# csukuangfj/kaldi-hmm-gmm

Hardware: AMD Instinct MI355X
Metric: frames/sec (whole node) per EM iter (align+acc-stats), 5k-pdf x 64-Gauss (higher is better)
Workload: dtype f32 via f16x2s

## Files before the change

### include/khg_hip.h

```cpp
#ifndef KHG_HIP_H_
#define KHG_HIP_H_
#include <stdint.h>

#ifdef __cplusplus
extern "C" {
#endif

#define KHG_OK 0
#define KHG_E_ARG (-1)
#define KHG_E_HIP (-2)
#define KHG_E_RUNTIME (-3)
#define KHG_E_UNSUPPORTED (-4)
#define KHG_MAX_DIM 512

typedef struct khg_ctx khg_ctx;
typedef struct khg_model khg_model;
typedef struct khg_tm khg_tm;
typedef struct khg_utts khg_utts;
typedef struct khg_accs khg_accs;

const char *khg_last_error(void);
int khg_version(void);

int khg_ctx_create(int device, void *stream, khg_ctx **out);
// ... 22 lines not shown
#define KHG_OPT_K2_PROF 9
#define KHG_OPT_K3_BUCKET 10
#define KHG_OPT_K3_FORM 11
#define KHG_OPT_K3_PHASE_B 12
#define KHG_OPT_K3_NY 13
#define KHG_OPT_DEBUG 14
#define KHG_OPT_K3_PHASE_A 15
#define KHG_OPT_K2_SPLIT 16
#define KHG_OPT_K2S_HUB 17
#define KHG_OPT_LAT_OPS_LDS 18
#define KHG_OPT_K1_LAUNCH 19
#define KHG_OPT_K1_PGRID 20
#define KHG_OPT_K1_PROF 21
#define KHG_OPT_K2_LADDER 22
#define KHG_OPT_K3_PLANES 23
#define KHG_OPT_COUNT 24
#define KHG_INFO_SCRATCH_BYTES 100
#define KHG_INFO_SCRATCH_BLOCKS 101
int khg_ctx_set_option(khg_ctx *ctx, int option, int value);
int khg_ctx_get_option(const khg_ctx *ctx, int option, int *value);
int khg_option_check(int option, int value);
int khg_option_from_env(const char *name, const char *text, int *option, int *value);

int khg_model_create(khg_ctx *ctx, int32_t num_pdfs, int32_t dim, const int32_t *gauss_off_h,
                     const float *gconsts_h, const float *means_invvars_h,
                     const float *inv_vars_h, khg_model **out);
int khg_model_destroy(khg_model *m);
int khg_model_invalidate(khg_model *m);

int khg_tm_create(khg_ctx *ctx, int32_t num_tids, const int32_t *id2pdf_h, khg_tm **out);
int khg_tm_set_trans_cost(khg_tm *tm, const float *trans_cost_h);
// ... 7 lines not shown
int khg_utts_destroy(khg_utts *u);
typedef struct khg_graph khg_graph;
int khg_graph_create(khg_ctx *ctx, const khg_tm *tm, int32_t num_states, int32_t start, const int64_t *arc_off_h,
                     const int32_t *ilabel_h, const int32_t *olabel_h, const float *weight_h,
                     const int32_t *nextstate_h, const float *final_h, khg_graph **out);
int khg_graph_destroy(khg_graph *g);
int khg_graph_info(const khg_graph *g, int64_t *num_states, int64_t *num_arcs, int32_t *num_pdfs,
                   int32_t *max_in_degree, int64_t *device_bytes);
int khg_utts_create_on_graph(khg_ctx *ctx, const khg_tm *tm, khg_graph *g, int32_t n_utt, int32_t dim,
                             const int64_t *frame_off_h, const float *feats_h, const float *feats_d, khg_utts **out);
int khg_utts_graph_bytes(const khg_utts *u, int64_t *bytes);
int khg_utts_num_pdfs(const khg_utts *u, int64_t *pdf_off_h );
int khg_utts_pdfs(const khg_utts *u, int32_t *pdfs_h );
int khg_utts_k2_plan(khg_ctx *ctx, const khg_utts *u, int32_t out[8]);
int khg_utts_k2_ladder(khg_ctx *ctx, const khg_utts *u, int32_t *out);
int khg_utts_k3_planes(const khg_utts *u, int64_t *bytes, int64_t *packs, int32_t *used);
int khg_utts_pdf_first(const khg_utts *u, int32_t *first_h );

int khg_loglikes(khg_ctx *ctx, const khg_model *m, khg_utts *u);
int khg_loglikes_reachable(khg_ctx *ctx, const khg_model *m, khg_utts *u);
int khg_loglikes_band(khg_ctx *ctx, const khg_model *m, khg_utts *u);
int khg_utts_pdf_last(const khg_utts *u, int32_t *last_h );
int khg_loglikes_layout(const khg_utts *u, int64_t *ll_off_h, int64_t *total);
int khg_loglikes_download(khg_ctx *ctx, const khg_utts *u, float *ll_h);
int khg_loglikes_upload(khg_ctx *ctx, khg_utts *u, const float *ll_h);
int khg_utts_set_pdf_list(khg_utts *u, int32_t n, const int32_t *pdfs_h);
int khg_utts_features_changed(khg_utts *u);

typedef struct {
  float beam;
// ... 460 lines not shown
```

### kaldi_hmm_gmm_amd/_lib.py

```python
import ctypes as C
import os

import numpy as np

_HERE = os.path.dirname(os.path.abspath(__file__))
LIB_PATH = os.environ.get("KHG_LIBRARY") or os.path.join(_HERE, "libkhg_hip.so")


class KhgError(RuntimeError):
    """Mirror of the reference's std::runtime_error -> Python RuntimeError (csrc/log.h:46-53)."""


def _load():
    if not os.path.exists(LIB_PATH):
        raise ImportError(
            f"{LIB_PATH} not found: build it with `python -c 'import __graft_entry__ as g; g.build()'` "
            "(hipcc --offload-arch=gfx950). kaldi_hmm_gmm_amd has no CPU fallback."
        )
    try:
        import torch
    except ImportError:
        pass
    return C.CDLL(LIB_PATH)

# ... 123 lines not shown
        C.c_int,
        [vp, vp, C.c_int32, C.c_int32, c_i64p, c_f32p, vp, c_i64p, c_i32p, c_i64p, c_i32p, c_i32p, c_f32p, c_i32p,
         c_f32p, C.POINTER(vp)],
    ),
    "khg_utts_destroy": (C.c_int, [vp]),
    "khg_graph_create": (C.c_int, [vp, vp, C.c_int32, C.c_int32, c_i64p, c_i32p, c_i32p, c_f32p, c_i32p, c_f32p, C.POINTER(vp)]),
    "khg_graph_destroy": (C.c_int, [vp]),
    "khg_graph_info": (C.c_int, [vp, c_i64p, c_i64p, c_i32p, c_i32p, c_i64p]),
    "khg_utts_create_on_graph": (C.c_int, [vp, vp, vp, C.c_int32, C.c_int32, c_i64p, c_f32p, vp, C.POINTER(vp)]),
    "khg_utts_graph_bytes": (C.c_int, [vp, c_i64p]),
    "khg_utts_num_pdfs": (C.c_int, [vp, c_i64p]),
    "khg_utts_pdfs": (C.c_int, [vp, c_i32p]),
    "khg_utts_k2_plan": (C.c_int, [vp, vp, c_i32p]),
    "khg_utts_k2_ladder": (C.c_int, [vp, vp, c_i32p]),
    "khg_utts_k3_planes": (C.c_int, [vp, c_i64p, c_i64p, c_i32p]),
    "khg_utts_pdf_first": (C.c_int, [vp, c_i32p]),
    "khg_loglikes": (C.c_int, [vp, vp, vp]),
    "khg_loglikes_reachable": (C.c_int, [vp, vp, vp]),
    "khg_loglikes_band": (C.c_int, [vp, vp, vp]),
    "khg_utts_pdf_last": (C.c_int, [vp, c_i32p]),
    "khg_loglikes_layout": (C.c_int, [vp, c_i64p, c_i64p]),
    "khg_loglikes_download": (C.c_int, [vp, vp, c_f32p]),
    "khg_loglikes_upload": (C.c_int, [vp, vp, c_f32p]),
    "khg_utts_set_pdf_list": (C.c_int, [vp, C.c_int32, c_i32p]),
    "khg_utts_features_changed": (C.c_int, [vp]),
    "khg_comm_info": (C.c_int, [vp, c_i32p, c_i32p, c_i32p]),
    "khg_align_config_default": (None, [C.POINTER(AlignConfigC)]),
    "khg_align": (C.c_int, [vp, vp, vp, C.POINTER(AlignConfigC), c_i32p, c_i32p, c_i64p, C.c_int64, c_f32p, c_i32p]),
    "khg_ali_upload": (C.c_int, [vp, vp, c_i32p]),
    "khg_lattice_faster_config_default": (None, [C.POINTER(LatticeFasterConfigC)]),
# ... 203 lines not shown
```

### kaldi_hmm_gmm_amd/csrc/khg_ctx_model.hip

```cpp
#include "khg_internal.hpp"

#include <mutex>
#include "khg_k1_loglikes.hip.inc"

static thread_local std::string g_err;
extern "C" const char* khg_last_error(void) { return g_err.c_str(); }
int khg_set_error(int code, const std::string& msg) { g_err = msg; return code; }
extern "C" int khg_version(void) { return 100; }

static std::mutex g_ctx_mu;
static std::vector<khg_ctx*> g_ctxs;
static constexpr size_t KHG_ARENA_BYTES = size_t(24) << 20;
void* arena_alloc(khg_ctx* ctx, size_t bytes) {
  KhgArena& a = ctx->arena;
  if (!a.dev) {
    if (a.cap == SIZE_MAX) return nullptr;
    void *d = nullptr, *h = nullptr;
    if (hipMalloc(&d, KHG_ARENA_BYTES) != hipSuccess || hipHostMalloc(&h, KHG_ARENA_BYTES, hipHostMallocDefault) != hipSuccess) {
      if (d) (void)hipFree(d);
      (void)hipGetLastError();
      a.cap = SIZE_MAX;
      return nullptr;
    }
    a.dev = static_cast<char*>(d); a.host = static_cast<char*>(h); a.cap = KHG_ARENA_BYTES; a.top = a.base = 256;
// ... 119 lines not shown
  int n = 0; std::string all;
  for (auto& t : c->timings) {
    float v = 0.0f;
    (void)hipEventElapsedTime(&v, t.e0, t.e1);
    if (n < cap && ms) ms[n] = v;
    all += t.name; all += '\n';
    (void)hipEventDestroy(t.e0); (void)hipEventDestroy(t.e1);
    ++n;
  }
  c->timings.clear();
  if (names && names_cap > 0) { size_t k = std::min<size_t>(all.size(), (size_t)names_cap - 1); memcpy(names, all.data(), k); names[k] = 0; }
  *n_out = n;
  return KHG_OK;
}
static const struct { int lo, hi; } k_opt_range[KHG_OPT_COUNT] = {
  {KHG_K1_AUTO, KHG_K1_F16X2S}, {0, 4}, {0, 6}, {0, 1 << 20}, {-1, 1}, {0, 255}, {0, 1}, {0, 4}, {0, 3}, {0, 1}, {0, 2}, {0, 2}, {0, 2}, {0, 64}, {0, 1}, {0, 1}, {0, 1}, {0, 1 << 20}, {0, 1}, {0, 2}, {0, 1 << 16}, {0, 1}, {0, 1}, {0, 2}};
extern "C" int khg_option_check(int opt, int value) {
  if (opt < 0 || opt >= KHG_OPT_COUNT) return khg_set_error(KHG_E_ARG, "khg_option_check: no such option");
  if (value < k_opt_range[opt].lo || value > k_opt_range[opt].hi || (opt == KHG_OPT_K1_FORM && value == 1))
    return khg_set_error(KHG_E_ARG, "khg_ctx_set_option: option " + std::to_string(opt) + " takes values " + std::to_string(k_opt_range[opt].lo) + " .. " + std::to_string(k_opt_range[opt].hi));
  return KHG_OK;
}
extern "C" int khg_ctx_set_option(khg_ctx* c, int opt, int value) {
  if (!c || opt < 0 || opt >= KHG_OPT_COUNT) return khg_set_error(KHG_E_ARG, "khg_ctx_set_option: bad arguments");
  int rc = khg_option_check(opt, value);
  if (rc) return rc;
  c->opt[opt] = value;
  return KHG_OK;
}
extern "C" int khg_ctx_get_option(const khg_ctx* c, int opt, int* value) {
  if (c && value && (opt == KHG_INFO_SCRATCH_BYTES || opt == KHG_INFO_SCRATCH_BLOCKS)) {
// ... 6 lines not shown
}
extern "C" int khg_ctx_set_k1_form(khg_ctx* c, int form) { return khg_ctx_set_option(c, KHG_OPT_K1_FORM, form); }
static const struct { const char* name; int opt; const char* words; } k_env_tab[] = {
  {"KHG_K1", KHG_OPT_K1_FORM, "auto=0,pdf=2,fp32=2,utt=3,f16x2=4,f16x2s=5"},
  {"KHG_K1_ORDER", KHG_OPT_K1_ORDER, "desc=0,none=1,asc=2,tiles=3,xcd=4"},
  {"KHG_K1_NF", KHG_OPT_K1_NF, ""}, {"KHG_K1P_TS", KHG_OPT_K1P_TS, ""}, {"KHG_K1_INTERLEAVE", KHG_OPT_K1_INTERLEAVE, ""},
  {"KHG_K1B_DBG", KHG_OPT_K1_DBG, ""}, {"KHG_K2_INORDER", KHG_OPT_K2_INORDER, ""}, {"KHG_K2_KS", KHG_OPT_K2_KS, ""},
  {"KHG_K2_SERIAL", KHG_OPT_K2_SERIAL, ""}, {"KHG_K2_PROF", KHG_OPT_K2_PROF, ""},
  {"KHG_K3_BUCKET", KHG_OPT_K3_BUCKET, "sort=0,atomic=1,count=2"}, {"KHG_K3_FORM", KHG_OPT_K3_FORM, "auto=0,block=1,valu=2"},
  {"KHG_K3_VALU", KHG_OPT_K3_FORM, "1=2"}, {"KHG_K3_PHASEB", KHG_OPT_K3_PHASE_B, "f64=0,f32=1,f16=2"},
  {"KHG_K3_NY", KHG_OPT_K3_NY, ""}, {"KHG_DEBUG", KHG_OPT_DEBUG, ""}, {"KHG_K3_PHASEA", KHG_OPT_K3_PHASE_A, "auto=0,f16=0,f32=1"},
  {"KHG_K2_SPLIT", KHG_OPT_K2_SPLIT, "on=0,off=1"}, {"KHG_K2S_HUB", KHG_OPT_K2S_HUB, ""},
  {"KHG_LAT_OPS_LDS", KHG_OPT_LAT_OPS_LDS, "on=0,off=1"},
  {"KHG_K1_LAUNCH", KHG_OPT_K1_LAUNCH, "auto=0,chunk=1,persistent=2"}, {"KHG_K1_PGRID", KHG_OPT_K1_PGRID, ""},
  {"KHG_K1_PROF", KHG_OPT_K1_PROF, ""}, {"KHG_K2_LADDER", KHG_OPT_K2_LADDER, "on=0,off=1"},
  {"KHG_K3_PLANES", KHG_OPT_K3_PLANES, "auto=0,off=1,on=2"}};
extern "C" int khg_option_from_env(const char* name, const char* text, int* option, int* value) {
  if (!name || !text || !*text || !option || !value) return khg_set_error(KHG_E_ARG, "khg_option_from_env: bad arguments");
  for (const auto& t : k_env_tab) {
    if (strcmp(t.name, name) != 0) continue;
    const char* e = text;
    int v = atoi(e);
    bool word = false;
    for (const char* w = t.words; *w;) {
      const char* eq = strchr(w, '=');
      const size_t n = (size_t)(eq - w);
      if (strlen(e) == n && strncmp(e, w, n) == 0) { v = atoi(eq + 1); word = true; break; }
      const char* comma = strchr(eq, ',');
      if (!comma) break;
      w = comma + 1;
    }
// ... 339 lines not shown
```

### kaldi_hmm_gmm_amd/csrc/khg_internal.hpp

```cpp
#pragma once
#include <hip/hip_runtime.h>

#include <algorithm>
#include <climits>
#include <cmath>
#include <cstdint>
#include <cstdio>
#include <cstdlib>
#include <cstring>
#include <deque>
#include <limits>
#include <string>
#include <type_traits>
#include <utility>
#include <vector>

#include "../../include/khg_hip.h"
#include "khg_dev_types.hip.inc"

int khg_set_error(int code, const std::string& msg);

#define HIPCHK(expr)                                                                         \
  do {                                                                                       \
    hipError_t e_ = (expr);                                                                  \
// ... 220 lines not shown
  K1sChunk* schunks_d = nullptr; int32_t n_schunks = 0, schunk_nmax = 0;
  K1sUnit* sunits_d = nullptr; std::vector<int32_t> sunits_pto; int sunits_reach = -1;
  uint8_t* bp_d = nullptr; int64_t *bp_off_d = nullptr, *path_off_d = nullptr, *words_off_d = nullptr;
  double* layer_best_d = nullptr; int32_t* layer_cnt_d = nullptr; int32_t* path_d = nullptr;
  unsigned char* k2_gscratch_d = nullptr; size_t k2_gscratch_bytes = 0;
  int32_t* k2_order_d = nullptr;
  int32_t *ali_d = nullptr, *words_d = nullptr, *num_words_d = nullptr, *status_d = nullptr;
  float* like_d = nullptr;
  bool ali_valid = false;
  char* out_blk_d = nullptr; size_t out_blk_bytes = 0;
  hipEvent_t ev_dp = nullptr, ev_ali = nullptr;
  bool ali_pending = false;
  int32_t *ali2_d = nullptr, *unc_d = nullptr, *unc_cnt_h = nullptr, *unc_cnt_dev = nullptr;
  int64_t* sub_off_d = nullptr;
  bool ali_split = false;
  int32_t *pdf_count_d = nullptr, *pdf_cursor_d = nullptr, *frame_ids_d = nullptr;
  uint32_t *sort_keys_d = nullptr, *sort_keys_out_d = nullptr, *sort_vals_d = nullptr; void* sort_tmp_d = nullptr; size_t sort_tmp_bytes = 0;
  int32_t* cs_hist_d = nullptr; size_t cs_hist_n = 0; int64_t* cs_tot_d = nullptr; size_t cs_tot_n = 0;
  double *k3_part_d = nullptr, *k3_llpart_d = nullptr; size_t k3_part_n = 0, k3_llpart_n = 0;
  void* k3_items_d = nullptr; int32_t* k3_item_off_d = nullptr; size_t k3_items_n = 0, k3_item_off_n = 0;
  int64_t* pdf_start_d = nullptr; unsigned long long* tid_count_d = nullptr;
  int32_t k3_P = 0, k3_tids = 0;
  void* k3x_d = nullptr; int64_t k3x_bytes = 0, k3x_packs = 0; std::vector<int32_t> k3x_key; bool k3x_used = false;
  int32_t *pe_row_d = nullptr, *pe_tid_d = nullptr, *pe_ids_d = nullptr; float* pe_w_d = nullptr; size_t pe_cap = 0;
  uint32_t *pe_keys_d = nullptr, *pe_keys_out_d = nullptr, *pe_vals_d = nullptr; void* pe_tmp_d = nullptr; size_t pe_tmp_bytes = 0;
  int64_t* pe_start_d = nullptr; int32_t pe_P = 0;
  uint64_t *rc_keys_d = nullptr, *rc_keys_out_d = nullptr; uint32_t *rc_vals_d = nullptr, *rc_vals_out_d = nullptr;
  int32_t *rc_flag_d = nullptr, *rc_inc_d = nullptr, *rc_row_d = nullptr; float* rc_cell_d = nullptr; size_t rc_cap = 0;
  void* rc_tmp_d = nullptr; size_t rc_tmp_bytes = 0;
  int32_t *rc_cell_start_d = nullptr, *rc_item_off_d = nullptr; int64_t* rc_stats_d = nullptr; int32_t rc_P = -1;
// ... 74 lines not shown
```

### kaldi_hmm_gmm_amd/csrc/khg_k2.hip

```cpp
#include "khg_internal.hpp"

#include "khg_k2_hashlist.hip.inc"
#include "khg_k2_viterbi.hip.inc"

extern "C" void khg_align_config_default(khg_align_config* c) {
  c->beam = 200.0f; c->retry_beam = 0.0f; c->careful = 0; c->acoustic_scale = 1.0f;
  c->max_active = INT32_MAX; c->min_active = 20; c->beam_delta = 0.5f; c->hash_ratio = 2.0f;
  c->like_scale = 0.0f;
}

static int ensure_ali(khg_ctx* ctx, khg_utts* u) {
  if (u->ali_d) return KHG_OK;
  if (u->small && u->has_graphs) {
    const size_t nu = (size_t)u->n_utt, nw = (size_t)u->words_off[u->n_utt];
    const size_t bytes = 4 * (3 * nu + nw + (size_t)u->N) + 64;
    int rc = u_alloc(u, &u->out_blk_d, bytes);
    if (rc) return rc;
    u->out_blk_bytes = bytes;
    int32_t* p = reinterpret_cast<int32_t*>(u->out_blk_d);
    u->status_d = p; u->like_d = reinterpret_cast<float*>(p + nu); u->num_words_d = p + 2 * nu; u->words_d = p + 3 * nu; u->ali_d = p + 3 * nu + nw;
    return KHG_OK;
  }
  return u_alloc(u, &u->ali_d, (size_t)u->N);
}
// ... 82 lines not shown
  if (!u->has_graphs) return khg_set_error(KHG_E_ARG, "khg_utts_k2_plan: the utterance set has no decoding graphs");
  const K2Plan p = k2_plan(ctx, u);
  out[0] = p.KS; out[1] = p.DEG; out[2] = p.FAST ? 1 : 0; out[3] = p.GMEM ? 1 : 0; out[4] = p.SC ? 1 : 0;
  out[5] = p.nthr; out[6] = p.GMEM ? 0 : (int32_t)p.lds_dp; out[7] = p.faithful;
  return KHG_OK;
}

extern "C" int khg_utts_k2_ladder(khg_ctx* ctx, const khg_utts* u, int32_t* out) {
  if (ctx_dead(ctx) || !u || !out) return khg_set_error(KHG_E_ARG, "khg_utts_k2_ladder: bad arguments");
  { int rf = utts_foreign_ctx(ctx, u, "khg_utts_k2_ladder"); if (rf) return rf; }
  if (!u->has_graphs) return khg_set_error(KHG_E_ARG, "khg_utts_k2_ladder: the utterance set has no decoding graphs");
  *out = k2_plan(ctx, u).LAD ? 1 : 0;
  return KHG_OK;
}

extern "C" int khg_align(khg_ctx* ctx, const khg_tm* tm, khg_utts* u, const khg_align_config* cfg,
                         int32_t* ali_h, int32_t* words_h, int64_t* words_off_h, int64_t words_cap,
                         float* like_h, int32_t* status_h) {
  if (ctx_dead(ctx) || !tm || !u || !cfg) return khg_set_error(KHG_E_ARG, "khg_align: bad arguments");
  { int rf = utts_foreign_ctx(ctx, u, "khg_align"); if (rf) return rf; }
  if (!u->has_graphs) return khg_set_error(KHG_E_ARG, "khg_align: the utterance set has no decoding graphs");
  if (!u->ll_valid) return khg_set_error(KHG_E_ARG, "khg_align: call khg_loglikes first");
  if (u->max_states > 65535)
    return khg_set_error(KHG_E_UNSUPPORTED, "khg_align: more than 65535 states in one decoding graph (" + std::to_string(u->max_states) + "); the aligner's limit");
  if (u->max_indeg > 254)
    return khg_set_error(KHG_E_UNSUPPORTED, "khg_align: a state has more than 254 incoming arcs (" + std::to_string(u->max_indeg) + "); the aligner's limit");
  if ((cfg->retry_beam != 0 && cfg->retry_beam <= cfg->beam) || cfg->beam <= 0.0)
    return khg_set_error(KHG_E_RUNTIME, "Beams do not make sense: beam " + std::to_string(cfg->beam) + ", retry-beam " + std::to_string(cfg->retry_beam));
  if (!(cfg->hash_ratio >= 1.0) || !(cfg->max_active > 1) || !(cfg->min_active >= 0 && cfg->min_active < cfg->max_active))
    return khg_set_error(KHG_E_RUNTIME, "FasterDecoderOptions assertion failed");
// ... 16 lines not shown
  }
  rc = arena_flush(ctx);
  if (rc) return rc;
  HIPCHK(hipMemsetAsync(u->ali_d, 0, sizeof(int32_t) * (size_t)u->N, ctx->stream));
  K2Args a;
  a.frame_off = u->frame_off_d; a.gidx = u->gidx_d; a.state_off = u->state_off_d; a.start = u->start_d;
  a.in_off = u->in_off_d; a.in_src = u->in_src_d; a.in_col = u->in_col_d; a.in_tid = u->in_tid_d;
  a.in_olabel = u->in_olabel_d; a.in_w = u->in_w_d; a.out_off = u->out_off_d; a.out_inidx = u->out_inidx_d;
  a.final_w = u->final_d; a.trans_cost = tm->has_trans_cost ? tm->trans_cost_d : nullptr;
  a.ll = u->ll_d; a.ll_off = u->ll_off_d;
  a.bp = u->bp_d; a.bp_off = u->bp_off_d; a.layer_best = u->layer_best_d; a.layer_cnt = u->layer_cnt_d;
  a.path = u->path_d; a.path_off = u->path_off_d;
  a.ali = u->ali_d; a.ali_fb = u->ali_d; a.unc = nullptr; a.unc_cnt = nullptr; a.words = u->words_d; a.words_off = u->words_off_d; a.num_words = u->num_words_d;
  a.like = u->like_d; a.status = u->status_d; a.err_flag = ctx->err_flag_d;
  a.prof = nullptr;
  if (!u->k2_order_d && u->n_utt > 1) {
    std::vector<int32_t> ord((size_t)u->n_utt);
    for (int i = 0; i < u->n_utt; ++i) ord[(size_t)i] = i;
    std::stable_sort(ord.begin(), ord.end(), [&](int32_t x, int32_t y) {
      return u->frame_off[x + 1] - u->frame_off[x] > u->frame_off[y + 1] - u->frame_off[y];
    });
    int rc2 = u_upload(ctx, u, &u->k2_order_d, ord);
    if (!rc2) rc2 = sync_pageable(ctx);
    if (rc2) return rc2;
  }
  a.order = ctx->opt[KHG_OPT_K2_INORDER] ? nullptr : u->k2_order_d;
  const bool split = !(ali_h || like_h || status_h || words_h) && u->n_utt > 64 && !u->small && ctx->opt[KHG_OPT_K2_SPLIT] == 0;
  if (split) {
    if (!u->ali2_d) {
      rc = u_alloc(u, &u->ali2_d, (size_t)u->N);
// ... 91 lines not shown
      if (plan.lds_f > 48 * 1024) HIPCHK(hipFuncSetAttribute((const void*)k2_viterbi_faithful<false>, hipFuncAttributeMaxDynamicSharedMemorySize, (int)plan.lds_f));
      KHG_LAUNCH(ctx, k2_viterbi_faithful<false>, dim3(u->n_utt), dim3(64), plan.lds_f, side, a);
    }
  }
  HIPCHK(hipGetLastError());
  if (!sync_call) { HIPCHK(hipEventRecord(u->ev_ali, side)); u->ali_pending = true; }
  u->ali_split = split;
  u->ali_valid = true;
  if (k2prof) {
    std::vector<long long> pr(16 * (size_t)u->n_utt);
    HIPCHK(hipStreamSynchronize(ctx->stream));
    HIPCHK(hipStreamSynchronize(side));
    HIPCHK(hipMemcpy(pr.data(), a.prof, pr.size() * 8, hipMemcpyDeviceToHost));
    (void)hipFree(a.prof);
    double ph[4] = {0, 0, 0, 0}, sT = 0, sS = 0, sf = 0; int n = 0;
    for (int i = 0; i < u->n_utt; ++i) if (pr[i * 8 + 4]) { for (int k = 0; k < 4; ++k) ph[k] += (double)(pr[i * 8 + k + 1] - pr[i * 8 + k]); sT += pr[i * 8 + 5]; sS += pr[i * 8 + 6]; sf += pr[i * 8 + 7]; ++n; }
    if (n) fprintf(stderr, "[KHG_K2_PROF] %d utts, avg T %.1f S %.1f fast %.2f threads %d lds %zu | ticks: setup %.0f forward %.0f traceback %.0f replay %.0f\n",
                   n, sT / n, sS / n, sf / n, nthr, lds_dp, ph[0] / n, ph[1] / n, ph[2] / n, ph[3] / n);
    const long long* pc = pr.data() + 8 * (size_t)u->n_utt;
    double cs[3] = {0, 0, 0}, cf = 0, cp[3] = {0, 0, 0}; int nc = 0;
    for (int i = 0; i < u->n_utt; ++i) if (pc[i * 8 + 3]) { for (int k = 0; k < 3; ++k) { cs[k] += (double)(pc[i * 8 + k + 1] - pc[i * 8 + k]); cp[k] += (double)pc[i * 8 + 5 + k]; } cf += (double)pc[i * 8 + 4]; ++nc; }
    if (nc) fprintf(stderr, "[KHG_K2_PROF] chain decoder: %d utts, avg frames decoded %.1f | ticks: setup %.0f frames %.0f (%.1f per frame: GetCutoff %.1f, pass 1 %.1f, pass 2 %.1f, rest = row flush + score staging) finish %.0f\n",
                    nc, cf / nc, cs[0] / nc, cs[1] / nc, cs[1] / std::max(1.0, cf), cp[0] / std::max(1.0, cf), cp[1] / std::max(1.0, cf), cp[2] / std::max(1.0, cf), cs[2] / nc);
  }
  if (!ali_h && !like_h && !status_h && !words_h) return KHG_OK;
  rc = wait_ali(ctx, u);
  if (rc) return rc;
  if (u->out_blk_d && ctx->arena.owns(u->out_blk_d)) {
    char* hm = ctx->arena.mirror(u->out_blk_d);
    HIPCHK(hipMemcpyAsync(hm, u->out_blk_d, u->out_blk_bytes, hipMemcpyDeviceToHost, ctx->stream));
    rc = check_err_flag(ctx, "khg_align");
    if (rc) return rc;
    const size_t nu = (size_t)u->n_utt, nwt = (size_t)u->words_off[u->n_utt];
// ... 72 lines not shown
```

### kaldi_hmm_gmm_amd/csrc/khg_k2_viterbi.hip.inc

```

struct K2Args {
  const int64_t* frame_off;
  const int32_t* gidx;
  const int64_t* state_off;
  const int32_t* start;
  const int64_t* in_off;
  const int32_t* in_src;
  const int32_t* in_col;
  const int32_t* in_tid;
  const int32_t* in_olabel;
  const float* in_w;
  const int64_t* out_off;
  const int32_t* out_inidx;
  const float* final_w;
  const float* trans_cost;
  const float* ll;
  const int64_t* ll_off;
  uint8_t* bp;
  const int64_t* bp_off;
  double* layer_best;
  int32_t* layer_cnt;
  int32_t* path;
  const int64_t* path_off;
  int32_t* ali;
// ... 1 lines not shown
  int32_t* unc;
  int32_t* unc_cnt;
  int32_t* words;
  const int64_t* words_off;
  int32_t* num_words;
  float* like;
  int32_t* status;
  int32_t* err_flag;
  long long* prof;
  float beam, retry_beam, acoustic_scale, like_scale, beam_delta, hash_ratio;
  int32_t max_active, min_active;
  int32_t max_states, max_inarcs;
  unsigned char* gscratch;
  int64_t gscratch_stride;
  const int32_t* order;
};

#ifndef K2_WAVES_PER_EU
#define K2_WAVES_PER_EU 5
#endif
#define K2_BP_NONE 255
#define K2_ST_NEED_FALLBACK 16

__device__ __forceinline__ unsigned long long k2_d2key(double d) {
  unsigned long long b = (unsigned long long)__double_as_longlong(d);
  return (b & 0x8000000000000000ull) ? ~b : (b | 0x8000000000000000ull);
}
__device__ __forceinline__ double k2_key2d(unsigned long long k) {
  unsigned long long b = (k & 0x8000000000000000ull) ? (k & 0x7fffffffffffffffull) : ~k;
  return __longlong_as_double((long long)b);
}

__device__ int k2_finish(const K2Args& a, int u, int best_state, const int32_t* s_in_off,
                         const int32_t* s_src, const int32_t* s_col, const float* s_w,
// ... 92 lines not shown
               "v_min_f32_dpp %0, %0, %0 row_bcast:15 row_mask:0xa bank_mask:0xf\n\ts_nop 1\n\t"
               "v_min_f32_dpp %0, %0, %0 row_bcast:31 row_mask:0xc bank_mask:0xf\n\ts_nop 1"
               : "+v"(v));
  return v;
}
__device__ __forceinline__ double k2_wave_min(double v) {
#pragma unroll
  for (int o = 32; o > 0; o >>= 1) { double t = __shfl_xor(v, o); v = t < v ? t : v; }
  return v;
}
template <int CTRL, int ROWMASK>
__device__ __forceinline__ double k2_dpp_d(double old, double v) {
  const int lo = __builtin_amdgcn_update_dpp(__double2loint(old), __double2loint(v), CTRL, ROWMASK, 0xf, false);
  const int hi = __builtin_amdgcn_update_dpp(__double2hiint(old), __double2hiint(v), CTRL, ROWMASK, 0xf, false);
  return __hiloint2double(hi, lo);
}
__device__ __forceinline__ int k2_wave_sum(int v) {
#pragma unroll
  for (int o = 32; o > 0; o >>= 1) v += __shfl_xor(v, o);
  return v;
}
__device__ __forceinline__ float k2_round_down(double d) {
  float f = (float)d;
  if ((double)f > d) f = __int_as_float(__float_as_int(f) + (f > 0.0f ? -1 : (f < 0.0f ? 1 : (int)0x80000001)));
  return f;
}

template <int DEG, int NB>
__device__ __forceinline__ void k2_decode_nibble(int nib, int& ord, int& tie) {
  if constexpr (DEG == 2) { ord = (nib & 1) ? 0 : ((nib & 2) ? 1 : (1 << NB) - 1); tie = (nib & 3) == 3 ? 1 : 0; }
// ... 471 lines not shown
      const unsigned* W = reinterpret_cast<const unsigned*>(bp);
      const uint32_t* arcw = reinterpret_cast<const uint32_t*>(s_arc);
      auto trace = [&](auto nslot_c) {
        constexpr int NSLOT = decltype(nslot_c)::value;
        int ioff[NSLOT];
        unsigned w[NSLOT], wn[NSLOT];
        int g = T >> 3;
#pragma unroll
        for (int q = 0; q < NSLOT; ++q) {
          const int sq = lane + 64 * q;
          ioff[q] = sq < S ? s_in_off[sq] : 0;
          w[q] = W[(int64_t)g * GW + min(sq, GW - 1)];
          wn[q] = 0u;
        }
        int sst = __builtin_amdgcn_readfirstlane(st);
        for (; g >= 0 && !bad; --g) {
          if (g > 0) {
#pragma unroll
            for (int q = 0; q < NSLOT; ++q) wn[q] = W[(int64_t)(g - 1) * GW + min(lane + 64 * q, GW - 1)];
          }
          int aiv[8][NSLOT], srcv[8][NSLOT];
#pragma unroll
          for (int k = 0; k < 8; ++k)
#pragma unroll
            for (int q = 0; q < NSLOT; ++q) {
              const int nib = (int)((w[q] >> (4 * k)) & 15u);
              int ord, tieb;
              k2_decode_nibble<DEG, NB>(nib, ord, tieb);
              const int none = ord == BNONE;
              const int ai = ioff[q] + (none ? 0 : ord);
// ... 86 lines not shown
      }
      hi = layer < 0 ? -1 : lo;
    }
    hi = __shfl(hi, 0); st = __shfl(st, 0); n = __shfl(n, 0); bad = __shfl(bad, 0); ptie = __shfl(ptie, 0);
    k2_lds_sync();
  }
  if (a.prof && tid == 0) a.prof[u * 8 + 3] = clock64();
  double cost = 0.0;
  float v1 = 0.0f, v2 = 0.0f;
  int t = 0, nw = 0;
  bool ok = !bad;
  const double beam = (double)a.beam;
  const int64_t wcap = a.words_off[u + 1] - a.words_off[u];
  int32_t* words = a.words + a.words_off[u];
  k2_global_sync();
  if (!bad) {
    ok = (0.0 < lbest[0] + beam) || lcnt[0] <= a.min_active;
    for (int base = n - 1; base >= 0; base -= 64) {
      const int idx = base - lane;
      int ai = 0, col = -1, tidl = 0, ol = 0; float w = 0.0f, ac = 0.0f;
      if (idx >= 0) {
        ai = path[idx];
        K2Arc ar = s_arc[ai];
        col = ar.col; w = ar.w;
        tidl = a.in_tid[in0 + ai];
        ol = a.in_olabel[in0 + ai];
      }
      const unsigned long long em = __ballot(idx >= 0 && col >= 0);
      const int before = __popcll(em & ((1ull << lane) - 1ull));
      const int tf = t + before;
      if (idx >= 0 && col >= 0) {
        ac = -1 * (a.acoustic_scale * llu[(int64_t)col * tpad + tf]);
        a.ali[f0 + tf] = tidl;
// ... 21 lines not shown
      const float tot_cost = (float)(ca - cb);
      const float ac_cost = tot_cost - w;
      if (__ballot(mine && !(ca < lb) && !small) != 0ull) ok = false;
      t += __popcll(em);
      {
        const unsigned long long wm = __ballot(mine && ol != 0);
        if (mine && ol != 0) { const int pos = nw + __popcll(wm & ((1ull << lane) - 1ull)); if (pos < wcap) words[pos] = ol; }
        nw += __popcll(wm);
      }
      for (int k = 0; k < cnt; ++k) {
        v1 = __int_as_float(__builtin_amdgcn_readlane(__float_as_int(w), k)) + v1;
        v2 = __int_as_float(__builtin_amdgcn_readlane(__float_as_int(ac_cost), k)) + v2;
      }
    }
  }
  if (a.prof && tid == 0) { a.prof[u * 8 + 4] = clock64(); a.prof[u * 8 + 5] = T; a.prof[u * 8 + 6] = S; a.prof[u * 8 + 7] = FAST; }
  int stt = 0;
  if (lane == 0) {
    if (bad || nw > wcap) {
      stt = K2_ST_NEED_FALLBACK;
    } else {
      v1 = a.final_w[s0 + best_state] + v1;
      v2 = 0.0f + v2;
      a.num_words[u] = nw;
      a.like[u] = -(v1 + v2) / a.like_scale;
      stt = (ok && !tie && !ptie && a.max_active == INT32_MAX) ? (KHG_ALIGN_DONE | KHG_ALIGN_EXACT_DP) : K2_ST_NEED_FALLBACK;
    }
    a.status[u] = stt;
  }
  if (a.unc) {
    stt = __builtin_amdgcn_readfirstlane(stt);
// ... 1140 lines not shown
```

### kaldi_hmm_gmm_amd/csrc/khg_pybind.cpp

```cpp
#include <chrono>

#include <pybind11/numpy.h>
#include <pybind11/pybind11.h>
#include <pybind11/stl.h>

#include <cstdint>
#include <cstring>
#include <limits>
#include <string>
#include <vector>

#include "../../include/khg_hip.h"
#include "khg_py_ebw.hpp"
#include "khg_py_lattices.hpp"

namespace py = pybind11;

namespace {

py::object g_khg_error;

void Check(int rc) {
  if (rc == KHG_OK) return;
  const char* msg = khg_last_error();
// ... 27 lines not shown
    void* st = stream.is_none() ? nullptr : reinterpret_cast<void*>(stream.cast<uintptr_t>());
    Check(khg_ctx_create(dev, st, &h));
  }
  ~KContext() { close(); }
  void close() { if (h) { khg_ctx_destroy(h); h = nullptr; } }
  void sync() { Check(NoGil([&] { return khg_ctx_sync(h); })); }
  void set_timing(bool on) { Check(khg_ctx_set_timing(h, on ? 1 : 0)); }
  void set_k1_form(const std::string& f) {
    int v = f == "auto" ? KHG_K1_AUTO : (f == "pdf" || f == "fp32") ? KHG_K1_FP32_PDF : f == "utt" ? KHG_K1_FP32_UTT : f == "f16x2" ? KHG_K1_F16X2 : f == "f16x2s" ? KHG_K1_F16X2S : -1;
    if (v < 0) throw py::key_error(f);
    Check(khg_ctx_set_k1_form(h, v));
  }
  static int opt_id(const py::object& o) {
    if (py::isinstance<py::int_>(o)) return o.cast<int>();
    static const char* names[KHG_OPT_COUNT] = {"k1_form", "k1_order", "k1_nf", "k1p_ts", "k1_interleave", "k1_dbg", "k2_inorder", "k2_ks", "k2_serial",
                                               "k2_prof", "k3_bucket", "k3_form", "k3_phase_b", "k3_ny", "debug", "k3_phase_a", "k2_split", "k2s_hub", "lat_ops_lds", "k1_launch", "k1_pgrid", "k1_prof", "k2_ladder", "k3_planes"};
    const std::string n = o.cast<std::string>();
    for (int i = 0; i < KHG_OPT_COUNT; ++i) if (n == names[i]) return i;
    if (n == "scratch_bytes") return KHG_INFO_SCRATCH_BYTES;
    if (n == "scratch_blocks") return KHG_INFO_SCRATCH_BLOCKS;
    throw py::key_error(n);
  }
  int get_option(py::object name) { int v = 0; Check(khg_ctx_get_option(h, opt_id(name), &v)); return v; }
  int set_option(py::object name, int value) {
    const int id = opt_id(name);
    int old = 0;
    Check(khg_ctx_get_option(h, id, &old));
    Check(khg_ctx_set_option(h, id, value));
    return old;
  }
  py::list timings() {
// ... 557 lines not shown
    d["nthr"] = o[5]; d["lds_bytes"] = o[6]; d["faithful_form"] = o[7];
    return d;
  }
  py::dict k3_planes() {
    int64_t bytes = 0, packs = 0; int32_t used = 0;
    Check(khg_utts_k3_planes(h, &bytes, &packs, &used));
    py::dict d;
    d["bytes"] = bytes; d["packs"] = packs; d["used"] = used != 0;
    return d;
  }
  bool k2_ladder(py::object ctx_o) {
    int32_t o = 0;
    Check(khg_utts_k2_ladder(ctx_o.cast<KContext*>()->h, h, &o));
    return o != 0;
  }
  py::object pdf_first_frames() {
    Arr<int64_t> off({(py::ssize_t)n_utt + 1});
    Check(khg_utts_num_pdfs(h, off.mutable_data()));
    const py::ssize_t n = off.at(n_utt);
    Arr<int32_t> first({n > 0 ? n : 1});
    Check(khg_utts_pdf_first(h, first.mutable_data()));
    return py::array(first)[py::slice(0, n, 1)];
  }
  py::object pdf_last_frames() {
    Arr<int64_t> off({(py::ssize_t)n_utt + 1});
    Check(khg_utts_num_pdfs(h, off.mutable_data()));
    const py::ssize_t n = off.at(n_utt);
    Arr<int32_t> last({n > 0 ? n : 1});
    Check(khg_utts_pdf_last(h, last.mutable_data()));
    return py::array(last)[py::slice(0, n, 1)];
// ... 395 lines not shown
      .def("allreduce_range", &KAccs::allreduce_range, py::arg("model"), py::arg("first_pdf"), py::arg("n_pdf"), py::arg("comm") = py::none())
      .def("split", &KAccs::split).def("relayout", &KAccs::relayout).def("download_range", &KAccs::download_range)
      .def("download_occ", [](KAccs& a) { return a.download_range(0, a.sumG); })
      .def("download_trans", &KAccs::download_trans).def("download", &KAccs::download).def("upload", &KAccs::upload)
      .def("add", &KAccs::add, py::arg("scale"), py::arg("src")).def("scale", &KAccs::scale, py::arg("f"))
      .def("smooth_with_accum", &KAccs::smooth_with_accum, py::arg("tau"), py::arg("src"), py::arg("model"), py::arg("count") = true)
      .def("close", &KAccs::close);

  py::class_<KUtts>(m, "UtteranceSet")
      .def(py::init<py::object, py::object, Arr<int64_t>, py::object, py::object, py::object, py::object>(), py::arg("ctx"), py::arg("tm"), py::arg("frame_off"),
           py::arg("feats"), py::arg("dim") = py::none(), py::arg("graphs") = py::none(), py::arg("graph") = py::none())
      .def_property_readonly("graph_bytes", [](KUtts& x) { int64_t b = 0; Check(khg_utts_graph_bytes(x.h, &b)); return b; })
      .def_property_readonly("h", [](KUtts& x) { return reinterpret_cast<uintptr_t>(x.h); })
      .def_readonly("ctx", &KUtts::ctx_obj).def_readonly("frame_off", &KUtts::frame_off).def_readonly("n_utt", &KUtts::n_utt)
      .def_readonly("dim", &KUtts::dim)
      .def("set_pdf_list", &KUtts::set_pdf_list).def("features_changed", &KUtts::features_changed).def("pdf_lists", &KUtts::pdf_lists).def("k2_plan", &KUtts::k2_plan, py::arg("ctx")).def("k2_ladder", &KUtts::k2_ladder, py::arg("ctx")).def("k3_planes", &KUtts::k3_planes).def("pdf_first_frames", &KUtts::pdf_first_frames)
      .def("pdf_last_frames", &KUtts::pdf_last_frames)
      .def("loglikes", &KUtts::loglikes, py::arg("model"), py::arg("reachable_only") = false, py::arg("band") = false)
      .def("loglikes_layout", &KUtts::loglikes_layout).def("download_loglikes", &KUtts::download_loglikes)
      .def("upload_loglikes", &KUtts::upload_loglikes)
      .def("align", &KUtts::align, py::arg("tm"), py::arg("beam") = 200.0f, py::arg("retry_beam") = 0.0f, py::arg("acoustic_scale") = 1.0f,
           py::arg("careful") = false, py::arg("max_active") = (int64_t)std::numeric_limits<int32_t>::max(), py::arg("min_active") = 20,
           py::arg("beam_delta") = 0.5f, py::arg("hash_ratio") = 2.0f, py::arg("download") = true)
      .def("decode_lattice_faster", &KUtts::decode_lattice_faster, py::arg("tm"), py::arg("beam") = 16.0f,
           py::arg("max_active") = std::numeric_limits<int32_t>::max(), py::arg("min_active") = 200, py::arg("lattice_beam") = 10.0f,
           py::arg("prune_interval") = 25, py::arg("beam_delta") = 0.5f, py::arg("hash_ratio") = 2.0f, py::arg("prune_scale") = 0.1f,
           py::arg("acoustic_scale") = 1.0f, py::arg("allow_partial") = true, py::arg("scratch_per_frame") = 0)
      .def("raw_lattice_faster", &KUtts::raw_lattice_faster, py::arg("tm"), py::arg("beam") = 16.0f,
           py::arg("max_active") = std::numeric_limits<int32_t>::max(), py::arg("min_active") = 200, py::arg("lattice_beam") = 10.0f,
           py::arg("prune_interval") = 25, py::arg("beam_delta") = 0.5f, py::arg("hash_ratio") = 2.0f, py::arg("prune_scale") = 0.1f,
           py::arg("acoustic_scale") = 1.0f, py::arg("allow_partial") = true, py::arg("scratch_per_frame") = 0)
// ... 281 lines not shown
```

Before: 449.2 million.

## Parallelize Viterbi traceback and replay cost accumulation with wave scans

Adds a branch-free traceback path for low in-degree graphs that precomputes source-state words per lane and walks 8 frames per word with readlane, avoiding per-frame LDS lookups. It also replaces the lane-serial cost replay with a wave-wide double prefix scan. The scan runs only when an exponent/magnitude bound shows the reassociated sum matches the serial float order, and otherwise falls back to the serial loop. Both paths are on by default and can be disabled with a new KHG_K2_TAIL option. Profiling now reports how many replay batches took the scanned path versus the serial one.

```diff
diff --git a/include/khg_hip.h b/include/khg_hip.h
--- a/include/khg_hip.h
+++ b/include/khg_hip.h
@@ -60,7 +60,8 @@
 #define KHG_OPT_K1_PROF 21
 #define KHG_OPT_K2_LADDER 22
 #define KHG_OPT_K3_PLANES 23
-#define KHG_OPT_COUNT 24
+#define KHG_OPT_K2_TAIL 24
+#define KHG_OPT_COUNT 25
 #define KHG_INFO_SCRATCH_BYTES 100
 #define KHG_INFO_SCRATCH_BLOCKS 101
 int khg_ctx_set_option(khg_ctx *ctx, int option, int value);
@@ -98,6 +99,7 @@
 int khg_utts_pdfs(const khg_utts *u, int32_t *pdfs_h );
 int khg_utts_k2_plan(khg_ctx *ctx, const khg_utts *u, int32_t out[8]);
 int khg_utts_k2_ladder(khg_ctx *ctx, const khg_utts *u, int32_t *out);
+int khg_utts_k2_tail(const khg_utts *u, int32_t *out, int64_t cap);
 int khg_utts_k3_planes(const khg_utts *u, int64_t *bytes, int64_t *packs, int32_t *used);
 int khg_utts_pdf_first(const khg_utts *u, int32_t *first_h );
 
diff --git a/kaldi_hmm_gmm_amd/_lib.py b/kaldi_hmm_gmm_amd/_lib.py
--- a/kaldi_hmm_gmm_amd/_lib.py
+++ b/kaldi_hmm_gmm_amd/_lib.py
@@ -161,6 +161,7 @@
     "khg_utts_k2_plan": (C.c_int, [vp, vp, c_i32p]),
     "khg_utts_k2_ladder": (C.c_int, [vp, vp, c_i32p]),
     "khg_utts_k3_planes": (C.c_int, [vp, c_i64p, c_i64p, c_i32p]),
+    "khg_utts_k2_tail": (C.c_int, [vp, c_i32p, C.c_int64]),
     "khg_utts_pdf_first": (C.c_int, [vp, c_i32p]),
     "khg_loglikes": (C.c_int, [vp, vp, vp]),
     "khg_loglikes_reachable": (C.c_int, [vp, vp, vp]),
diff --git a/kaldi_hmm_gmm_amd/csrc/khg_ctx_model.hip b/kaldi_hmm_gmm_amd/csrc/khg_ctx_model.hip
--- a/kaldi_hmm_gmm_amd/csrc/khg_ctx_model.hip
+++ b/kaldi_hmm_gmm_amd/csrc/khg_ctx_model.hip
@@ -157,7 +157,7 @@
   return KHG_OK;
 }
 static const struct { int lo, hi; } k_opt_range[KHG_OPT_COUNT] = {
-  {KHG_K1_AUTO, KHG_K1_F16X2S}, {0, 4}, {0, 6}, {0, 1 << 20}, {-1, 1}, {0, 255}, {0, 1}, {0, 4}, {0, 3}, {0, 1}, {0, 2}, {0, 2}, {0, 2}, {0, 64}, {0, 1}, {0, 1}, {0, 1}, {0, 1 << 20}, {0, 1}, {0, 2}, {0, 1 << 16}, {0, 1}, {0, 1}, {0, 2}};
+  {KHG_K1_AUTO, KHG_K1_F16X2S}, {0, 4}, {0, 6}, {0, 1 << 20}, {-1, 1}, {0, 255}, {0, 1}, {0, 4}, {0, 3}, {0, 1}, {0, 2}, {0, 2}, {0, 2}, {0, 64}, {0, 1}, {0, 1}, {0, 1}, {0, 1 << 20}, {0, 1}, {0, 2}, {0, 1 << 16}, {0, 1}, {0, 1}, {0, 2}, {0, 1}};
 extern "C" int khg_option_check(int opt, int value) {
   if (opt < 0 || opt >= KHG_OPT_COUNT) return khg_set_error(KHG_E_ARG, "khg_option_check: no such option");
   if (value < k_opt_range[opt].lo || value > k_opt_range[opt].hi || (opt == KHG_OPT_K1_FORM && value == 1))
@@ -194,7 +194,7 @@
   {"KHG_LAT_OPS_LDS", KHG_OPT_LAT_OPS_LDS, "on=0,off=1"},
   {"KHG_K1_LAUNCH", KHG_OPT_K1_LAUNCH, "auto=0,chunk=1,persistent=2"}, {"KHG_K1_PGRID", KHG_OPT_K1_PGRID, ""},
   {"KHG_K1_PROF", KHG_OPT_K1_PROF, ""}, {"KHG_K2_LADDER", KHG_OPT_K2_LADDER, "on=0,off=1"},
-  {"KHG_K3_PLANES", KHG_OPT_K3_PLANES, "auto=0,off=1,on=2"}};
+  {"KHG_K3_PLANES", KHG_OPT_K3_PLANES, "auto=0,off=1,on=2"}, {"KHG_K2_TAIL", KHG_OPT_K2_TAIL, "on=0,off=1"}};
 extern "C" int khg_option_from_env(const char* name, const char* text, int* option, int* value) {
   if (!name || !text || !*text || !option || !value) return khg_set_error(KHG_E_ARG, "khg_option_from_env: bad arguments");
   for (const auto& t : k_env_tab) {
diff --git a/kaldi_hmm_gmm_amd/csrc/khg_internal.hpp b/kaldi_hmm_gmm_amd/csrc/khg_internal.hpp
--- a/kaldi_hmm_gmm_amd/csrc/khg_internal.hpp
+++ b/kaldi_hmm_gmm_amd/csrc/khg_internal.hpp
@@ -258,6 +258,7 @@
   int32_t *ali2_d = nullptr, *unc_d = nullptr, *unc_cnt_h = nullptr, *unc_cnt_dev = nullptr;
   int64_t* sub_off_d = nullptr;
   bool ali_split = false;
+  std::vector<int32_t> k2_tail;
   int32_t *pdf_count_d = nullptr, *pdf_cursor_d = nullptr, *frame_ids_d = nullptr;
   uint32_t *sort_keys_d = nullptr, *sort_keys_out_d = nullptr, *sort_vals_d = nullptr; void* sort_tmp_d = nullptr; size_t sort_tmp_bytes = 0;
   int32_t* cs_hist_d = nullptr; size_t cs_hist_n = 0; int64_t* cs_tot_d = nullptr; size_t cs_tot_n = 0;
diff --git a/kaldi_hmm_gmm_amd/csrc/khg_k2.hip b/kaldi_hmm_gmm_amd/csrc/khg_k2.hip
--- a/kaldi_hmm_gmm_amd/csrc/khg_k2.hip
+++ b/kaldi_hmm_gmm_amd/csrc/khg_k2.hip
@@ -120,6 +120,14 @@
   return KHG_OK;
 }
 
+extern "C" int khg_utts_k2_tail(const khg_utts* u, int32_t* out, int64_t cap) {
+  if (!u || !out) return khg_set_error(KHG_E_ARG, "khg_utts_k2_tail: bad arguments");
+  if (u->k2_tail.empty()) return khg_set_error(KHG_E_ARG, "khg_utts_k2_tail: no khg_align under KHG_OPT_K2_PROF on this set yet");
+  if (cap < (int64_t)u->k2_tail.size()) return khg_set_error(KHG_E_ARG, "khg_utts_k2_tail: cap too small");
+  std::copy(u->k2_tail.begin(), u->k2_tail.end(), out);
+  return KHG_OK;
+}
+
 extern "C" int khg_align(khg_ctx* ctx, const khg_tm* tm, khg_utts* u, const khg_align_config* cfg,
                          int32_t* ali_h, int32_t* words_h, int64_t* words_off_h, int64_t words_cap,
                          float* like_h, int32_t* status_h) {
@@ -166,6 +174,7 @@
   a.ali = u->ali_d; a.ali_fb = u->ali_d; a.unc = nullptr; a.unc_cnt = nullptr; a.words = u->words_d; a.words_off = u->words_off_d; a.num_words = u->num_words_d;
   a.like = u->like_d; a.status = u->status_d; a.err_flag = ctx->err_flag_d;
   a.prof = nullptr;
+  a.tail_off = ctx->opt[KHG_OPT_K2_TAIL];
   if (!u->k2_order_d && u->n_utt > 1) {
     std::vector<int32_t> ord((size_t)u->n_utt);
     for (int i = 0; i < u->n_utt; ++i) ord[(size_t)i] = i;
@@ -287,9 +296,15 @@
     HIPCHK(hipMemcpy(pr.data(), a.prof, pr.size() * 8, hipMemcpyDeviceToHost));
     (void)hipFree(a.prof);
     double ph[4] = {0, 0, 0, 0}, sT = 0, sS = 0, sf = 0; int n = 0;
-    for (int i = 0; i < u->n_utt; ++i) if (pr[i * 8 + 4]) { for (int k = 0; k < 4; ++k) ph[k] += (double)(pr[i * 8 + k + 1] - pr[i * 8 + k]); sT += pr[i * 8 + 5]; sS += pr[i * 8 + 6]; sf += pr[i * 8 + 7]; ++n; }
-    if (n) fprintf(stderr, "[KHG_K2_PROF] %d utts, avg T %.1f S %.1f fast %.2f threads %d lds %zu | ticks: setup %.0f forward %.0f traceback %.0f replay %.0f\n",
-                   n, sT / n, sS / n, sf / n, nthr, lds_dp, ph[0] / n, ph[1] / n, ph[2] / n, ph[3] / n);
+    for (int i = 0; i < u->n_utt; ++i) if (pr[i * 8 + 4]) { for (int k = 0; k < 4; ++k) ph[k] += (double)(pr[i * 8 + k + 1] - pr[i * 8 + k]); sT += pr[i * 8 + 5]; sS += pr[i * 8 + 6]; sf += (double)(pr[i * 8 + 7] & 0xff); ++n; }
+    u->k2_tail.assign(2 * (size_t)u->n_utt, 0);
+    long long bs = 0, bl = 0;
+    for (int i = 0; i < u->n_utt; ++i) {
+      u->k2_tail[2 * (size_t)i] = (int32_t)((pr[i * 8 + 7] >> 8) & 0xffffff); u->k2_tail[2 * (size_t)i + 1] = (int32_t)(pr[i * 8 + 7] >> 32);
+      bs += u->k2_tail[2 * (size_t)i]; bl += u->k2_tail[2 * (size_t)i + 1];
+    }
+    if (n) fprintf(stderr, "[KHG_K2_PROF] %d utts, avg T %.1f S %.1f fast %.2f threads %d lds %zu | ticks: setup %.0f forward %.0f traceback %.0f replay %.0f | replay batches: %lld scanned, %lld serial\n",
+                   n, sT / n, sS / n, sf / n, nthr, lds_dp, ph[0] / n, ph[1] / n, ph[2] / n, ph[3] / n, bs, bl);
     const long long* pc = pr.data() + 8 * (size_t)u->n_utt;
     double cs[3] = {0, 0, 0}, cf = 0, cp[3] = {0, 0, 0}; int nc = 0;
     for (int i = 0; i < u->n_utt; ++i) if (pc[i * 8 + 3]) { for (int k = 0; k < 3; ++k) { cs[k] += (double)(pc[i * 8 + k + 1] - pc[i * 8 + k]); cp[k] += (double)pc[i * 8 + 5 + k]; } cf += (double)pc[i * 8 + 4]; ++nc; }
diff --git a/kaldi_hmm_gmm_amd/csrc/khg_k2_viterbi.hip.inc b/kaldi_hmm_gmm_amd/csrc/khg_k2_viterbi.hip.inc
--- a/kaldi_hmm_gmm_amd/csrc/khg_k2_viterbi.hip.inc
+++ b/kaldi_hmm_gmm_amd/csrc/khg_k2_viterbi.hip.inc
@@ -39,10 +39,17 @@
   unsigned char* gscratch;
   int64_t gscratch_stride;
   const int32_t* order;
+  int32_t tail_off;
 };
 
 #ifndef K2_WAVES_PER_EU
 #define K2_WAVES_PER_EU 5
+#endif
+#ifndef K2_TAIL_TRACE
+#define K2_TAIL_TRACE 1
+#endif
+#ifndef K2_TAIL_REPLAY
+#define K2_TAIL_REPLAY 1
 #endif
 #define K2_BP_NONE 255
 #define K2_ST_NEED_FALLBACK 16
@@ -165,6 +172,28 @@
   const int lo = __builtin_amdgcn_update_dpp(__double2loint(old), __double2loint(v), CTRL, ROWMASK, 0xf, false);
   const int hi = __builtin_amdgcn_update_dpp(__double2hiint(old), __double2hiint(v), CTRL, ROWMASK, 0xf, false);
   return __hiloint2double(hi, lo);
+}
+__device__ __forceinline__ double k2_wave_scand(double v) {
+  v += k2_dpp_d<0x111, 0xf>(0.0, v);
+  v += k2_dpp_d<0x112, 0xf>(0.0, v);
+  v += k2_dpp_d<0x114, 0xf>(0.0, v);
+  v += k2_dpp_d<0x118, 0xf>(0.0, v);
+  v += k2_dpp_d<0x142, 0xa>(0.0, v);
+  v += k2_dpp_d<0x143, 0xc>(0.0, v);
+  return v;
+}
+__device__ __forceinline__ double k2_readlane_d(double v, int l) {
+  return __hiloint2double(__builtin_amdgcn_readlane(__double2hiint(v), l), __builtin_amdgcn_readlane(__double2loint(v), l));
+}
+__device__ __forceinline__ double k2_wave_sumd(double v) { return k2_readlane_d(k2_wave_scand(v), 63); }
+__device__ __forceinline__ unsigned k2_wave_minu(unsigned v) {
+  v = min(v, (unsigned)__builtin_amdgcn_update_dpp(-1, (int)v, 0x111, 0xf, 0xf, false));
+  v = min(v, (unsigned)__builtin_amdgcn_update_dpp(-1, (int)v, 0x112, 0xf, 0xf, false));
+  v = min(v, (unsigned)__builtin_amdgcn_update_dpp(-1, (int)v, 0x114, 0xf, 0xf, false));
+  v = min(v, (unsigned)__builtin_amdgcn_update_dpp(-1, (int)v, 0x118, 0xf, 0xf, false));
+  v = min(v, (unsigned)__builtin_amdgcn_update_dpp(-1, (int)v, 0x142, 0xa, 0xf, false));
+  v = min(v, (unsigned)__builtin_amdgcn_update_dpp(-1, (int)v, 0x143, 0xc, 0xf, false));
+  return (unsigned)__builtin_amdgcn_readlane((int)v, 63);
 }
 __device__ __forceinline__ int k2_wave_sum(int v) {
 #pragma unroll
@@ -666,6 +695,66 @@
           wn[q] = 0u;
         }
         int sst = __builtin_amdgcn_readfirstlane(st);
+        if constexpr (K2_TAIL_TRACE && DEG <= 3 && KS == 1) {
+          if (!a.tail_off) {
+            constexpr int NBITS = NB + 1;
+            int srcr[NSLOT][DEG], srcx[NSLOT][DEG];
+#pragma unroll
+            for (int q = 0; q < NSLOT; ++q) {
+              const int sq = lane + 64 * q;
+              const int ib = sq < S ? s_in_off[sq] : 0, ie = sq < S ? s_in_off[sq + 1] : 0;
+#pragma unroll
+              for (int j = 0; j < DEG; ++j) srcr[q][j] = ib + j < ie ? (int)((arcw[2 * (ib + j)] & 0xffffu) << NBITS) : 0;
+#pragma unroll
+              for (int j = 0; j + 1 < DEG; ++j) srcx[q][j] = srcr[q][j] ^ srcr[q][DEG - 1];
+            }
+            for (; g >= 0 && !bad; --g) {
+              if (g > 0) {
+#pragma unroll
+                for (int q = 0; q < NSLOT; ++q) wn[q] = W[(int64_t)(g - 1) * GW + min(lane + 64 * q, GW - 1)];
+              }
+              int pk[8][NSLOT];
+#pragma unroll
+              for (int k = 0; k < 8; ++k)
+#pragma unroll
+                for (int q = 0; q < NSLOT; ++q) {
+                  const int nib = (int)((w[q] >> (4 * k)) & (unsigned)((1 << NBITS) - 1));
+                  int sel = srcr[q][0];
+                  if constexpr (DEG == 2) sel = srcr[q][1] ^ (srcx[q][0] & -(nib & 1));
+                  if constexpr (DEG == 3) { const int o = nib & BNONE; sel = srcr[q][2] ^ (srcx[q][0] & -(int)(o == 0)) ^ (srcx[q][1] & -(int)(o == 1)); }
+                  pk[k][q] = sel | nib;
+                }
+              int pv = 0, cnt = 0;
+#pragma unroll
+              for (int k = 7; k >= 0; --k) {
+                const int L = 8 * g + k;
+                if (L <= T && L >= 1 && !bad) {
+                  const int q = sst >> 6, l = sst & 63;
+                  int pw = __builtin_amdgcn_readlane(pk[k][0], l);
+#pragma unroll
+                  for (int qq = 1; qq < NSLOT; ++qq)
+                    if (q == qq) pw = __builtin_amdgcn_readlane(pk[k][qq], l);
+                  int ord, tieb;
+                  k2_decode_nibble<DEG, NB>(pw & ((1 << NBITS) - 1), ord, tieb);
+                  if (ord == BNONE) {
+                    bad = 1;
+                  } else {
+                    ptie |= tieb;
+                    pv = lane == cnt ? ((sst << NBITS) | ord) : pv;
+                    ++cnt;
+                    sst = pw >> NBITS;
+                  }
+                }
+              }
+              if (lane < cnt) path[n + lane] = s_in_off[pv >> NBITS] + (pv & BNONE);
+              n += cnt;
+#pragma unroll
+              for (int q = 0; q < NSLOT; ++q) w[q] = wn[q];
+            }
+            st = sst;
+            return;
+          }
+        }
         for (; g >= 0 && !bad; --g) {
           if (g > 0) {
 #pragma unroll
@@ -782,9 +871,88 @@
   const int64_t wcap = a.words_off[u + 1] - a.words_off[u];
   int32_t* words = a.words + a.words_off[u];
   k2_global_sync();
-  if (!bad) {
+  int nscan = 0, nserial = 0;
+  bool replayed = false;
+  if constexpr (FAST && K2_TAIL_REPLAY) {
+    if (!bad && !a.tail_off) {
+      replayed = true;
+      ok = (0.0 < lbest[0] + beam) || lcnt[0] <= a.min_active;
+      unsigned emin1 = 0xffffffffu;
+      double sumabs = 0.0;
+      bool serial = false;
+      f32x2 vv = {0.0f, 0.0f};
+      for (int base = n - 1; base >= 0; base -= 64) {
+        const int idx = base - lane;
+        const bool mine = idx >= 0;
+        int ai = 0, col = 0, tidl = 0, ol = 0; float w = 0.0f, ac = 0.0f;
+        if (mine) {
+          ai = path[idx];
+          K2Arc ar = s_arc[ai];
+          col = ar.col; w = ar.w;
+          tidl = a.in_tid[in0 + ai];
+          ol = a.in_olabel[in0 + ai];
+        }
+        const int tf = t + lane;
+        if (mine) {
+          ac = -1 * (a.acoustic_scale * llu[(int64_t)col * tpad + tf]);
+          a.ali[f0 + tf] = tidl;
+        }
+        const int cnt = base >= 63 ? 64 : base + 1;
+        const int tl = tf + (mine ? 1 : 0);
+        double lb = 0.0; int small = 0;
+        if (mine) {
+          lb = lbest[tl] + beam;
+          small = lcnt[tl] <= a.min_active && (tl == 0 || lcnt[tl - 1] <= a.min_active);
+        }
+        const double cost_in = cost;
+        double ca = 0.0;
+        if (!serial) {
+          const unsigned aw = __float_as_uint(w) & 0x7fffffffu, aa = __float_as_uint(ac) & 0x7fffffffu;
+          const unsigned m1 = k2_wave_minu(min(aw - 1u, aa - 1u));
+          emin1 = min(emin1, m1);
+          sumabs += k2_wave_sumd((double)__uint_as_float(aw) + (double)__uint_as_float(aa));
+          const unsigned eb = (emin1 + 1u) >> 23;
+          const double bound = __hiloint2double((int)((eb + 925u) << 20), 0);
+          serial = !((emin1 == 0xffffffffu || eb >= 27u) && sumabs <= bound);
+        }
+        if (!serial) {
+          ++nscan;
+          double d = (double)w + (double)ac;
+          d = lane == 0 ? cost_in + d : d;
+          ca = k2_wave_scand(d);
+          cost = k2_readlane_d(ca, cnt - 1);
+        } else {
+          ++nserial;
+          for (int k = 0; k < cnt; ++k) {
+            const float wk = __int_as_float(__builtin_amdgcn_readlane(__float_as_int(w), k));
+            const float ack = __int_as_float(__builtin_amdgcn_readlane(__float_as_int(ac), k));
+            const double ncost = (cost + wk) + ack;
+            ca = lane == k ? ncost : ca;
+            cost = ncost;
+          }
+        }
+        const double cb = k2_dpp_d<0x138, 0xf>(cost_in, ca);
+        const float tot_cost = (float)(ca - cb);
+        const float ac_cost = tot_cost - w;
+        if (__ballot(mine && !(ca < lb) && !small) != 0ull) ok = false;
+        t += cnt;
+        {
+          const unsigned long long wm = __ballot(mine && ol != 0);
+          if (mine && ol != 0) { const int pos = nw + __popcll(wm & ((1ull << lane) - 1ull)); if (pos < wcap) words[pos] = ol; }
+          nw += __popcll(wm);
+        }
+        for (int k = 0; k < cnt; ++k) {
+          const f32x2 r = {__int_as_float(__builtin_amdgcn_readlane(__float_as_int(w), k)), __int_as_float(__builtin_amdgcn_readlane(__float_as_int(ac_cost), k))};
+          vv = r + vv;
+        }
+      }
+      v1 = vv[0]; v2 = vv[1];
+    }
+  }
+  if (!bad && !replayed) {
     ok = (0.0 < lbest[0] + beam) || lcnt[0] <= a.min_active;
     for (int base = n - 1; base >= 0; base -= 64) {
+      ++nserial;
       const int idx = base - lane;
       int ai = 0, col = -1, tidl = 0, ol = 0; float w = 0.0f, ac = 0.0f;
       if (idx >= 0) {
@@ -836,7 +1004,7 @@
       }
     }
   }
-  if (a.prof && tid == 0) { a.prof[u * 8 + 4] = clock64(); a.prof[u * 8 + 5] = T; a.prof[u * 8 + 6] = S; a.prof[u * 8 + 7] = FAST; }
+  if (a.prof && tid == 0) { a.prof[u * 8 + 4] = clock64(); a.prof[u * 8 + 5] = T; a.prof[u * 8 + 6] = S; a.prof[u * 8 + 7] = (long long)FAST | ((long long)nscan << 8) | ((long long)nserial << 32); }
   int stt = 0;
   if (lane == 0) {
     if (bad || nw > wcap) {
diff --git a/kaldi_hmm_gmm_amd/csrc/khg_pybind.cpp b/kaldi_hmm_gmm_amd/csrc/khg_pybind.cpp
--- a/kaldi_hmm_gmm_amd/csrc/khg_pybind.cpp
+++ b/kaldi_hmm_gmm_amd/csrc/khg_pybind.cpp
@@ -65,7 +65,7 @@
   static int opt_id(const py::object& o) {
     if (py::isinstance<py::int_>(o)) return o.cast<int>();
     static const char* names[KHG_OPT_COUNT] = {"k1_form", "k1_order", "k1_nf", "k1p_ts", "k1_interleave", "k1_dbg", "k2_inorder", "k2_ks", "k2_serial",
-                                               "k2_prof", "k3_bucket", "k3_form", "k3_phase_b", "k3_ny", "debug", "k3_phase_a", "k2_split", "k2s_hub", "lat_ops_lds", "k1_launch", "k1_pgrid", "k1_prof", "k2_ladder", "k3_planes"};
+                                               "k2_prof", "k3_bucket", "k3_form", "k3_phase_b", "k3_ny", "debug", "k3_phase_a", "k2_split", "k2s_hub", "lat_ops_lds", "k1_launch", "k1_pgrid", "k1_prof", "k2_ladder", "k3_planes", "k2_tail"};
     const std::string n = o.cast<std::string>();
     for (int i = 0; i < KHG_OPT_COUNT; ++i) if (n == names[i]) return i;
     if (n == "scratch_bytes") return KHG_INFO_SCRATCH_BYTES;
@@ -653,6 +653,11 @@
     Check(khg_utts_k2_ladder(ctx_o.cast<KContext*>()->h, h, &o));
     return o != 0;
   }
+  py::array k2_tail() {
+    Arr<int32_t> o({(py::ssize_t)n_utt, (py::ssize_t)2});
+    Check(khg_utts_k2_tail(h, o.mutable_data(), 2 * (int64_t)n_utt));
+    return o;
+  }
   py::object pdf_first_frames() {
     Arr<int64_t> off({(py::ssize_t)n_utt + 1});
     Check(khg_utts_num_pdfs(h, off.mutable_data()));
@@ -1078,7 +1083,7 @@
       .def_property_readonly("h", [](KUtts& x) { return reinterpret_cast<uintptr_t>(x.h); })
       .def_readonly("ctx", &KUtts::ctx_obj).def_readonly("frame_off", &KUtts::frame_off).def_readonly("n_utt", &KUtts::n_utt)
       .def_readonly("dim", &KUtts::dim)
-      .def("set_pdf_list", &KUtts::set_pdf_list).def("features_changed", &KUtts::features_changed).def("pdf_lists", &KUtts::pdf_lists).def("k2_plan", &KUtts::k2_plan, py::arg("ctx")).def("k2_ladder", &KUtts::k2_ladder, py::arg("ctx")).def("k3_planes", &KUtts::k3_planes).def("pdf_first_frames", &KUtts::pdf_first_frames)
+      .def("set_pdf_list", &KUtts::set_pdf_list).def("features_changed", &KUtts::features_changed).def("pdf_lists", &KUtts::pdf_lists).def("k2_plan", &KUtts::k2_plan, py::arg("ctx")).def("k2_ladder", &KUtts::k2_ladder, py::arg("ctx")).def("k3_planes", &KUtts::k3_planes).def("k2_tail", &KUtts::k2_tail).def("pdf_first_frames", &KUtts::pdf_first_frames)
       .def("pdf_last_frames", &KUtts::pdf_last_frames)
       .def("loglikes", &KUtts::loglikes, py::arg("model"), py::arg("reachable_only") = false, py::arg("band") = false)
       .def("loglikes_layout", &KUtts::loglikes_layout).def("download_loglikes", &KUtts::download_loglikes)
```

New measurement: 460.7 million (median of 6 runs). 1.03x the previous value.
